# fverdoja/Fast-3D-Pointcloud-Segmentation

Measured on AMD Instinct MI355X. Metric: Mpoints/sec segmented end-to-end, 1M-pt RGB-D frames, higher is better.
Workload: dtype f32

## Files before the change

fast-3d-pointcloud-segmentation_amd/csrc/f3ds_hip.hip:

```cpp
#include <hip/hip_runtime.h>

#include <algorithm>
#include <cmath>
#include <atomic>
#include <map>
#include <chrono>
#include <cstdio>
#include <cstdlib>
#include <cstring>
#include <string>
#include <type_traits>
#include <mutex>
#include <set>
#include <vector>

#include "../../include/f3ds.h"
#include "f3ds_algo.h"
#include "f3ds_glasbey.h"
#include "f3ds_eval.h"
#include "f3ds_dev.h"
#include "f3ds_levels.h"
#include "f3ds_eval_levels.h"
#include "f3ds_rgbd.h"
#include "f3ds_track.h"
// ... 19 lines not shown
#define HIPCHECK(expr) do { hipError_t e_ = (expr); if (e_ != hipSuccess) { g_last_hip_error = std::string(#expr) + ": " + hipGetErrorString(e_); return F3DS_ERR_HIP; } } while (0)

template <class... Ts> struct ArgPack;
template <> struct ArgPack<> {};
template <class T, class... Ts> struct ArgPack<T, Ts...> { T head; ArgPack<Ts...> tail; };

template <class K, class... Done>
__device__ __forceinline__ void unpack_call(const ArgPack<>&, Done... d) { K{}(d...); }
template <class K, class T, class... Ts, class... Done>
__device__ __forceinline__ void unpack_call(const ArgPack<T, Ts...>& p, Done... d) { unpack_call<K>(p.tail, d..., p.head); }

template <class K, class = void> struct waves_per_simd { static constexpr int v = 1; };
template <class K> struct waves_per_simd<K, std::void_t<decltype(K::WAVES_PER_SIMD)>> { static constexpr int v = K::WAVES_PER_SIMD; };
template <class K, class = void> struct is_latency_kernel { static constexpr bool v = false; };
template <class K> struct is_latency_kernel<K, std::void_t<decltype(K::LATENCY_KERNEL)>> { static constexpr bool v = K::LATENCY_KERNEL; };
template <class K, class Pack>
__global__ __launch_bounds__(K::BLOCK, waves_per_simd<K>::v) void k_batched(const Pack* frames) {
#ifndef F3DS_EXP_NO_LATENCY_PRIO
    if constexpr (is_latency_kernel<K>::v) __builtin_amdgcn_s_setprio(3);
#endif
    const Pack p = frames[f3ds_frame()];
    unpack_call<K>(p);
}

template <class F> struct op_traits;
template <class C, class... Ps> struct op_traits<void (C::*)(Ps...) const> { using pack = ArgPack<std::decay_t<Ps>...>; };
template <class K> using pack_of = typename op_traits<decltype(&K::operator())>::pack;

inline void fill_pack(ArgPack<>&) {}
template <class T, class... Ts, class A, class... As>
inline void fill_pack(ArgPack<T, Ts...>& p, A a, As... as) {
    static_assert(std::is_convertible<A, T>::value && !(std::is_pointer<T>::value && std::is_integral<A>::value),
                  "rec<K>(): an argument does not convert implicitly to the kernel's parameter type (wrong element type, swapped arguments?)");
    p.head = a; fill_pack(p.tail, as...);
}

typedef hipError_t (*LaunchFn)(uint32_t gx, uint32_t nf, uint32_t lds, hipStream_t st, const void* dargs);
template <class K>
hipError_t launch_fn(uint32_t gx, uint32_t nf, uint32_t lds, hipStream_t st, const void* dargs) {
    using Pack = pack_of<K>;
    if (lds > 48u * 1024u) {
        hipError_t e = hipFuncSetAttribute(reinterpret_cast<const void*>(k_batched<K, Pack>), hipFuncAttributeMaxDynamicSharedMemorySize, (int)lds);
        if (e != hipSuccess) return e;
    }
    hipLaunchKernelGGL((k_batched<K, Pack>), dim3(gx ? gx : 1u, nf), dim3(K::BLOCK), lds, st, static_cast<const Pack*>(dargs));
    return hipGetLastError();
}
struct Cmd { LaunchFn fn; uint32_t gx, lds, bytes, off; };

const int g_inc_shift = [] { const char* e = dev_getenv("F3DS_INC_SHIFT"); return e ? atoi(e) : 6; }();

struct Switches {
    bool direct_labels = false, copy_stream = true, copy_duplex = false, split_voxel_accum = false, sweep_tiles = true, merge_spec = true, force_global_merge = false, no_stream_pool = false, sort_pairs = false, host_prof = false, trace_err = false, vox_hash = true, vox_tiles_forced = false, levels_global = false;
    int normals_threads = 0, merge_nw = 0, merge_keys = -1; uint32_t tile_holes = 0, ilist_slack = 32, r_rounds = F3DS_R_ROUNDS, grid_cap = 0, rgc_first_cap = 0; long relabel_lds_cap = -1;
    void read() {
        auto on = [](const char* n) { return dev_getenv(n) != nullptr; };
        auto num = [](const char* n, long dflt) { const char* e = dev_getenv(n); return e ? atol(e) : dflt; };
        direct_labels = num("F3DS_DIRECT_LABELS", 0) != 0; copy_stream = num("F3DS_COPY_STREAM", 1) != 0; copy_duplex = num("F3DS_COPY_STREAM", 1) == 2; split_voxel_accum = on("F3DS_SPLIT_VOXEL_ACCUM"); sweep_tiles = num("F3DS_SWEEP_TILES", 1) != 0; merge_spec = num("F3DS_MERGE_SPEC", 1) != 0;
        force_global_merge = on("F3DS_FORCE_GLOBAL_MERGE"); no_stream_pool = on("F3DS_NO_STREAM_POOL"); sort_pairs = on("F3DS_SORT_PAIRS");
        host_prof = on("F3DS_HOST_PROF"); trace_err = on("F3DS_TRACE_ERR");
        vox_tiles_forced = num("F3DS_VOX_TILES", 1) == 2;
        vox_hash = num("F3DS_VOX_TILES", 1) != 0 && !sort_pairs && !split_voxel_accum;
        normals_threads = (int)num("F3DS_NORMALS_THREADS", 0); tile_holes = (uint32_t)num("F3DS_SWEEP_TILE_HOLES", 0);
        { const long v = num("F3DS_MERGE_NW", 0); merge_nw = v == 4 ? 4 : (v ? 8 : 0); }
        { const char* e = dev_getenv("F3DS_MERGE_KEYS"); merge_keys = !e ? -1 : (!strcmp(e, "lds") ? 2 : (!strcmp(e, "global") ? 1 : 0)); }
        relabel_lds_cap = num("F3DS_RELABEL_LDS_CAP", -1);
        levels_global = num("F3DS_LEVELS_GLOBAL", 0) != 0;
        { const long v = num("F3DS_R_ROUNDS_RUN", F3DS_R_ROUNDS); r_rounds = v >= 1 && v <= F3DS_R_ROUNDS ? (uint32_t)v : (uint32_t)F3DS_R_ROUNDS; }
        { const long v = num("F3DS_ILIST_SLACK", 32); ilist_slack = v >= 1 && v <= 32 ? (uint32_t)v : 32u; }
        { const long v = num("F3DS_GRID_CAP", 0); grid_cap = v >= 1 && v <= 2048 ? (uint32_t)v : 0u; }
        { const long v = num("F3DS_RGC_FIRST_CAP", 0); rgc_first_cap = v >= 1 && v <= 0x7fffffffl ? (uint32_t)v : 0u; }
    }
};
thread_local Switches g_sw;
const int g_merge_shared_res = [] { const char* e = dev_getenv("F3DS_MERGE_SHARED_RES"); return e && atoi(e) == 2 ? 2 : 0; }();

#define F3DS_SCRATCH(X) \
    X(P16, pts)  X(unsigned char, img_depth) X(unsigned char, img_color) X(P16, spts) X(uint64_t, keys0) X(uint64_t, keys1) X(uint32_t, vals0) X(uint32_t, vals1) X(uint32_t, flags) X(uint32_t, incl) X(uint32_t, tiles) X(uint32_t, hist) X(uint32_t, seg_start) X(int, pt_voxel) X(uint32_t, labels) \
    X(uint32_t, vkey) X(uint32_t, vcount) X(float, vf) X(int, nbr) X(int, nbrT) X(uint64_t, hkeys) X(uint32_t, hvals) X(float, boxes) X(uint32_t, ckey) X(uint32_t, cell_start) X(uint64_t, chk) X(uint32_t, chv) X(uint32_t, chvals) X(int, seed_orig) X(uint32_t, keep) X(int, seed_kept) \
    X(uint32_t, owner0) X(uint32_t, ownR) X(float, dist0) X(unsigned char, R) X(float, hc) X(uint32_t, hcount) X(uint32_t, hlo) X(uint32_t, hhi) X(int, ghost_vox) X(unsigned char, ghost_active) X(unsigned char, ghost_done) X(uint32_t, ghost_head) X(uint32_t, ghost_next) \
    X(uint32_t, loff) X(float, rows) X(int, row_voxel) X(float, racc0) X(uint32_t, rcnt0) X(float, rrec0) X(unsigned char, ralive0) X(uint64_t, ehk) X(uint64_t, ekeys0) X(uint64_t, ekeys1) X(uint32_t, evals0) X(uint32_t, evals1) X(uint32_t, ea0) X(uint32_t, eb0) \
    X(uint32_t, ea) X(uint32_t, eb) X(float, ew) X(uint32_t, eku) X(int, ehist) X(unsigned char, ealive) X(uint32_t, ev_epoch) X(uint32_t, ev_key) X(int, ev_prev) X(float, racc) X(uint32_t, rcnt) X(float, rrec) X(unsigned char, ralive) X(uint32_t, rhead) X(uint32_t, rtail) X(uint32_t, lnext) X(uint32_t, parent) X(uint32_t, markA) X(uint32_t, markB) X(uint32_t, tl) X(uint32_t, merges) \
     X(float, r_vf) X(uint32_t, r_owner) X(float, r_dist) X(float, r_hc) X(uint32_t, r_hcount) X(uint32_t, r_hlo) X(uint32_t, r_hhi) X(int, r_gvox) X(unsigned char, r_gact) X(unsigned char, r_gdone) X(uint32_t, r_ghead) X(uint32_t, r_gnext) X(uint32_t, r_tl) X(uint32_t, r_tcnt) X(int, r_seed) X(uint32_t, r_L) \
    X(uint32_t, tstamp) X(uint32_t, tround) X(uint32_t, hdirty) X(uint32_t, htiles) X(uint32_t, htcnt) X(uint32_t, vwl) X(uint32_t, vwl2) X(uint32_t, vtmask) \
     X(uint32_t, glut) X(uint32_t, truth_pts) X(uint32_t, tsum) X(uint32_t, tcol) X(uint32_t, tlab) X(uint32_t, ctab) X(uint32_t, csize) X(uint32_t, eroot) X(uint32_t, eincl) \
     X(uint32_t, hcnt) X(uint32_t, pslot) X(uint32_t, vlist) \
     X(uint32_t, u_src) X(uint32_t, u_voff) X(float, u_xyz) X(uint32_t, u_rgba) X(float, u_cent) X(float, u_nrm) \
    X(float, deltas) X(uint64_t, skeys0) X(uint64_t, skeys1) X(uint32_t, svals0) X(uint32_t, svals1) X(uint32_t, cdf_hist) X(float, cdf) X(uint32_t, root) X(uint32_t, rincl) X(uint32_t, rrank) X(uint2, pool) X(uint32_t, rstart) X(uint32_t, rnleaf) X(uint32_t, rcap) X(uint32_t, tile_n1) X(uint32_t, tile_ord) X(uint32_t, tile_slots) X(uint32_t, ilist) X(uint32_t, istart) X(uint32_t, ilen) X(uint32_t, icap) \
     X(uint32_t, lv_into) X(uint32_t, lv_at) X(uint32_t, lv_pfx) X(float, lv_thr) X(uint32_t, lv_tab) X(uint32_t, lv_nreg) X(uint32_t, lv_out) \
     \
    X(uint64_t, evl_k0) X(uint64_t, evl_k1) X(uint32_t, evl_v0) X(uint32_t, evl_v1) X(uint32_t, evl_flag) X(uint64_t, evl_bkey) X(uint32_t, evl_bcnt) X(uint64_t, evl_ukey) X(uint32_t, evl_ucnt) X(uint32_t, evl_glist) \
    X(uint32_t, evl_ssize) X(unsigned char, evl_used) X(float, evl_hterm) X(float, evl_mterm) X(float, evl_tterm) X(uint32_t, evl_tsize) X(uint32_t, evl_order) X(uint32_t, evl_slot) X(uint32_t, evl_counts) X(uint32_t, evl_out) \
     \
    X(uint32_t, trk_lab) X(uint32_t, trk_end) X(uint32_t, trk_out) X(uint32_t, trk_id) X(uint32_t, trk_tid) \
     \
    X(unsigned char, rgt_depth) X(unsigned char, rgt_color) X(uint32_t, rgt_lab) X(RgAcc, rgt_acc) X(unsigned char, rgt_out) \
     \
    X(unsigned char, rgc_depth) X(uint32_t, rgc_lab) X(uint64_t, rgc_k0) X(uint64_t, rgc_k1) X(uint32_t, rgc_v0) X(uint32_t, rgc_v1) X(uint32_t, rgc_rec) X(uint32_t, rgc_flag) X(uint64_t, rgc_ukey) X(uint32_t, rgc_ustart) X(uint32_t, rgc_uend) X(uint32_t, rgc_cnt) X(unsigned char, rgc_out) \
     \
    X(unsigned char, rgs_depth) X(uint32_t, rgs_lab) X(ShAcc, rgs_acc) X(unsigned char, rgs_out) \
     \
    X(unsigned char, rgk_depth) X(uint32_t, rgk_lab) X(uint32_t, rgk_parent) X(uint32_t, rgk_cnt) X(uint32_t, rgk_flag) X(unsigned char, rgk_out)
template <class T> struct Scratch { T* p = nullptr; size_t cap = 0; int slot = -1; };
#define F3DS_SCRATCH_SLOT(T, name) S_##name,
#define F3DS_SCRATCH_MEMBER(T, name) Scratch<T> name{nullptr, 0, S_##name};
#define F3DS_SCRATCH_VISIT(T, name) if (const int rc_ = f(name)) return rc_;
enum ScratchSlot { F3DS_SCRATCH(F3DS_SCRATCH_SLOT) N_SCRATCH };

}

struct f3ds_ctx {
    int device = 0;
    hipStream_t own_stream = nullptr;
    hipStream_t stream = nullptr;
    hipEvent_t ev[11] = {};
    DevCounters* d_dc = nullptr;
    DevCounters* h_dc = nullptr;
    GridInfo* d_grid = nullptr;
    GridInfo* h_grid = nullptr;
    SeedGrid* d_sgrid = nullptr;
    std::vector<Cmd> cmds;
    std::vector<unsigned char> blob;
    std::vector<uintptr_t> pend;
// ... 482 lines not shown
    } else {
        rec<d_helper_own>(c, grid_for(S0, 256), 0u, sb.seeds, S0, owner0);
        rec<d_helper_init>(c, grid_for(S0 + 1, 256), 0u, sb.seeds, S0, owner0, ghost_vox, ghost_active, ghost_done, hlo, hhi, hcount, hc, tl, tcnt);
    }
    const int* nbrT = c->nbrT.p; const float* vf = sb.vf;
    SweepFrame a;
    a.sv = SweepView{(int)V, nbrT, vf, owner0, dist0, hc, ghost_head, ghost_next, &c->d_dc->n_ghosts, prm.seed_res, prm.w_normal, prm.w_color, prm.w_spatial, c->nbr.p};
    a.R = R; a.ownR = ownR; a.owner_out = owner0; a.dist_out = dist0;
    a.ghost_done = ghost_done; a.ghost_active = ghost_active; a.ghost_vox = ghost_vox; a.ghost_head = ghost_head; a.ghost_next = ghost_next;
    a.hlo = hlo; a.hhi = hhi; a.hcount = hcount; a.hc = hc; a.dc = c->d_dc; a.S0 = S0;
    a.tR0 = tiles4; a.tR1 = tiles4 + T; a.tC0 = tiles4 + 2 * (size_t)T; a.tC1 = tiles4 + 3 * (size_t)T; a.tRr = trr; a.hD = hD; a.T = T; a.tl = tl; a.tcnt = tcnt; a.wl = wl; a.wl2 = wl2; a.tmask = tmask;
    a.thr = a_sweep_thr(V, g_inc_shift);
    if (!g_sw.sweep_tiles) a.tile_n1 = nullptr;
    else a.tile_n1 = c->tile_n1.p;
    a.tile_ord = c->tile_ord.p; a.tile_slots = c->tile_slots.p;
    for (uint32_t t = 0; t < c->res.sweeps; ++t) {
        if (a_sweep_needs_clear(t)) rec_fill(c, R, 0u, V);
        rec<d_sweep_begin>(c, 1u, 0u, a, t);
        const bool can_skip = t >= 2u;
        const bool rounds = g_inc_shift >= 0 && can_skip;
        const uint32_t nrounds = rounds ? g_sw.r_rounds : 0u;
        rec<d_sweep_R_first>(c, grid_for(V, 256), 0u, a, a_sweep_tag(t), t, nrounds);
        for (uint32_t r = 1; r < nrounds; ++r) rec<d_sweep_R_round>(c, grid_for(V, 256), 0u, a, t, r, nrounds);
        for (uint32_t pass = 0; pass < F3DS_R_PASSES; ++pass) rec<d_sweep_R>(c, pass == 0 ? grid_for(V, 256) : 64u, 0u, a, a_sweep_tag(t), t, pass);
        rec<d_sweep_R_tail>(c, 1u, 0u, a, a_sweep_tag(t), t);
        rec<d_sweep_claim>(c, grid_for(V, 256), 0u, a, t);
        rec<d_centroid>(c, grid_for((size_t)S0 * 64u, 256), 0u, a, t);
    }
    return F3DS_OK;
}
int seg_sweeps(f3ds_ctx* c) {
    SweepBufs sb{&c->owner0, &c->dist0, &c->hc, &c->hcount, &c->hlo, &c->hhi, &c->ghost_vox, &c->ghost_active, &c->ghost_done, &c->ghost_head, &c->ghost_next, &c->htiles, &c->htcnt, c->vf.p, c->seed_kept.p, false};
    return seg_sweeps_on(c, sb);
}
int seg_supervoxels(f3ds_ctx* c) {
    const uint32_t V = c->V, S0 = c->S0;
    uint32_t *loff, *rcnt0, *ev0, *ev1; float *rows, *racc0, *rrec0; int* row_voxel; unsigned char* ralive0; uint64_t *ehk, *ek0, *ek1;
    ENSURE(c->loff, S0 + 2, loff);
    int rc = scan_u32(c, c->hcount.p, loff + 1, S0 + 1);
    if (rc) return rc;
    rec_fill(c, loff, 0u, 4);
    ENSURE(c->rows, ((size_t)V + S0 + 1) * 12, rows); ENSURE(c->row_voxel, (size_t)V + S0 + 1, row_voxel);
    ENSURE(c->racc0, (size_t)(S0 + 1) * 12, racc0); ENSURE(c->rcnt0, S0 + 1, rcnt0); ENSURE(c->rrec0, (size_t)(S0 + 1) * 16, rrec0);
    ENSURE(c->ralive0, S0 + 1, ralive0);
    rec_fill(c, ralive0, 0u, S0 + 1);
    rec_fill(c, rcnt0, 0u, (size_t)(S0 + 1) * 4);
    rec<d_sv_fill>(c, S0 ? (S0 + 3u) / 4u : 1u, 0u,
                   c->vf.p, c->owner0.p, S0, c->hlo.p, c->hhi.p, c->ghost_vox.p, c->ghost_active.p, c->hcount.p, loff, c->hc.p, rows, row_voxel, racc0, rcnt0, rrec0, ralive0, c->d_dc, c->htiles.p, c->htcnt.p, V);
    const uint32_t ecap = (uint32_t)std::min<uint64_t>((uint64_t)S0 * c->edge_mult + 1024u, 0x7fffffffu);
    const uint32_t ehcap = pow2_ge((size_t)ecap * 2);
    ENSURE(c->ehk, ehcap, ehk);
    ENSURE(c->ekeys0, ecap, ek0); ENSURE(c->ekeys1, ecap, ek1); ENSURE(c->evals0, ecap, ev0); ENSURE(c->evals1, ecap, ev1);
    rec_fill(c, ehk, 0xFFFFFFFFu, (size_t)ehcap * 8);
    rec<d_edges>(c, grid_for(V, 256), 0u, V, S0, c->nbrT.p, c->owner0.p, ehk, ehcap - 1, ek0, ecap, c->d_dc);
    rec<d_edges_ghost>(c, grid_for(S0, 256), 0u, V, S0, c->ghost_vox.p, c->ghost_active.p, c->nbrT.p, c->owner0.p, ehk, ehcap - 1, ek0, ecap, c->d_dc);
    return F3DS_OK;
}
int seg_edge_sort(f3ds_ctx* c, int sort_bits) {
    const uint32_t E = c->E, S0 = c->S0;
    uint32_t *ea0, *eb0; ENSURE(c->ea0, E, ea0); ENSURE(c->eb0, E, eb0);
    uint32_t* evs;
    { uint32_t* h; ENSURE(c->hist, (size_t)RS_BINS * (((size_t)E * 2 + RS_TILE - 1) / RS_TILE + 1), h); }
    rec<d_iota>(c, grid_for(E, 256), 0u, c->evals0.p, E);
    int rc = radix_sort(c, c->ekeys0.p, c->evals0.p, c->ekeys1.p, c->evals1.p, E, sort_bits, &c->eks, &evs);
    if (rc) return rc;
    rec<d_edge_init>(c, grid_for(E, 256), 0u, c->eks, E, S0, ea0, eb0);
    return F3DS_OK;
}
bool merge_il_layout(uint32_t E, uint32_t S0, int nw, int res, MergeLds* xl) {
    memset(xl, 0, sizeof *xl);
    if ((uint64_t)E * (res == 2 ? 10u : 2u) > (1u << 22)) return false;
    const MergeIlLayout L = merge_il_offsets(E, nw, res);
    xl->Ecap = L.Ecap; xl->NGcap = L.NGcap; xl->lds_bytes = L.total; xl->keys_in_lds = res;
    xl->spec = g_sw.merge_spec ? 1 : 0;
    return L.total <= MC_LDS_LIMIT && S0 <= 65534u;
}
enum MergeKind { MK_GLOBAL = 0, MK_IL = 1 };
inline int mk_waves(int kind) { return (kind - MK_IL) >= 2 ? 4 : 8; }
inline int mk_res(int kind) { return (kind - MK_IL) % 2 ? 0 : 2; }
int choose_merge_kind(const std::vector<f3ds_ctx*>& fr, bool force_global) {
    if (force_global || g_sw.force_global_merge) return MK_GLOBAL;
    const bool e_keys = g_sw.merge_keys >= 0;
    const bool shared = fr.size() >= 16 && g_batch_calls[fr[0]->device & 15].load(std::memory_order_relaxed) >= 2;
    const int nw = g_sw.merge_nw ? (g_sw.merge_nw == 8 ? 8 : 4) : (shared ? 4 : 8);
    const int first = e_keys ? (g_sw.merge_keys == 2 ? 2 : 0) : (shared ? g_merge_shared_res : 2);
    for (int res = first; res >= (e_keys ? first : 0); res -= 2) {
        bool ok = true;
        for (f3ds_ctx* c : fr) { MergeLds t; if (!merge_il_layout(c->E, c->S0, nw, res, &t)) { ok = false; break; } }
        if (ok) return MK_IL + (nw == 8 ? 0 : 2) + (res == 2 ? 0 : 1);
    }
    return MK_GLOBAL;
}
int seg_cluster_front(f3ds_ctx* c, const f3ds_params* prm, int kind) {
    const bool use_lds = kind != MK_GLOBAL;
    const uint32_t S0 = c->S0, E = c->E;
    float lambda = 0.5f; int bins = 500;
    if (prm->merging == F3DS_MANUAL_LAMBDA && prm->lambda != 0) { if (prm->lambda < 0 || prm->lambda > 1) return F3DS_ERR_RANGE; lambda = prm->lambda; }
    if (prm->merging == F3DS_EQUALIZATION && prm->bins != 0) { if (prm->bins < 0) return F3DS_ERR_RANGE; bins = (short)prm->bins; }
    if (prm->merging < 0 || prm->merging > 2 || prm->color_metric < 0 || prm->color_metric > 1 || prm->geom_metric < 0 || prm->geom_metric > 1) return F3DS_ERR_ARG;
    MergeDev m;
    memset(&m, 0, sizeof m);
    m.E = E; m.S0 = S0; m.threshold = prm->threshold; m.dc = c->d_dc;
    { const uint64_t cap = (uint64_t)E * c->ev_mult + 4096u; m.ev_cap = cap > 0x7fffffffull ? 0x7fffffffu : (uint32_t)cap; }
    ENSURE(c->ea, E, m.ea); ENSURE(c->eb, E, m.eb); ENSURE(c->ew, ((size_t)E + 2047) & ~(size_t)2047, m.ew);  ENSURE(c->eku, ((size_t)E + 2047) & ~(size_t)2047, m.eku);
    ENSURE(c->ehist, E, m.ehist); ENSURE(c->ealive, E, m.ealive);
    ENSURE(c->ev_epoch, m.ev_cap, m.ev_epoch); ENSURE(c->ev_key, m.ev_cap, m.ev_key); ENSURE(c->ev_prev, m.ev_cap, m.ev_prev);
    ENSURE(c->racc, (size_t)(S0 + 1) * 12, m.racc); ENSURE(c->rrec, (size_t)(S0 + 1) * 16, m.rrec);
    ENSURE(c->rcnt, S0 + 1, m.rcnt); ENSURE(c->ralive, S0 + 1, m.ralive);
// ... 1793 lines not shown
```

fast-3d-pointcloud-segmentation_amd/csrc/f3ds_kernels.inc:

```


namespace {

struct P16 { float x, y, z; uint32_t rgba; };

struct DevCounters {
    unsigned long long n_finite;
    uint32_t bbox[6];
    uint32_t bbox_any;
    uint32_t n_valid;
    uint32_t n_voxels;
    uint32_t n_cells;
    uint32_t n_seeds;
    uint32_t n_edges;
    uint32_t n_alive;
    uint32_t n_merges;
    uint32_t n_regions;
    uint32_t n_events;
    int error;
    int r_overflow;
    float lambda;
    uint32_t seg_count;
    uint32_t n_ghosts;
    int depth;
// ... 1784 lines not shown
            }
            __syncthreads();
        }
        if (threadIdx.x == 0) seed[h - 1u] = sv[0];
    }
};
struct d_reseed_own {
    static constexpr int BLOCK = 256;
    __device__ void operator()(const int* seed, uint32_t S0, uint32_t* owner) const {
        for (uint32_t i = BIX * blockDim.x + threadIdx.x; i < S0; i += gridDim.x * blockDim.x) if (seed[i] >= 0) atomicMax(&owner[seed[i]], i + 1u);
    }
};
struct d_reseed_init {
    static constexpr int BLOCK = 256;
    __device__ void operator()(const int* seed, uint32_t S0, const uint32_t* owner, int* ghost_vox, unsigned char* ghost_active, unsigned char* ghost_done, uint32_t* hlo,
                               uint32_t* hhi, uint32_t* hcount, uint32_t* tl, uint32_t* tcnt) const {
        for (uint32_t i = BIX * blockDim.x + threadIdx.x; i <= S0; i += gridDim.x * blockDim.x) {
            ghost_done[i] = 0;
            const int v = i == 0u ? -1 : seed[i - 1];
            if (v < 0) { ghost_vox[i] = -1; ghost_active[i] = 0; hlo[i] = 0; hhi[i] = 0; hcount[i] = 0; tcnt[i] = 0; continue; }
            const bool ghost = owner[v] != i;
            ghost_vox[i] = ghost ? v : -1;
            ghost_active[i] = ghost ? 1 : 0;
            hlo[i] = (uint32_t)v; hhi[i] = (uint32_t)v; hcount[i] = 1;
            tl[(size_t)i * HT_CAP] = (uint32_t)v >> 6; tcnt[i] = ghost ? 0u : 1u;
        }
    }
};
struct SweepFrame {
    SweepView sv;
    unsigned char* R; uint32_t* ownR;
    uint32_t* owner_out; float* dist_out;
    unsigned char *ghost_done, *ghost_active; int* ghost_vox; uint32_t *ghost_head, *ghost_next;
    uint32_t *hlo, *hhi, *hcount; float* hc; DevCounters* dc; uint32_t S0;
    uint32_t *tR0, *tR1, *tC0, *tC1;
    uint32_t* tRr;
    uint32_t* hD;
    uint32_t *tl, *tcnt;
    uint32_t *wl, *wl2;
    uint32_t* tmask;
    uint32_t T, thr;
    const uint32_t *tile_n1, *tile_ord, *tile_slots;
    __device__ uint32_t* tR_this(uint32_t t) const { return (t & 1u) ? tR1 : tR0; }
    __device__ uint32_t* tC_this(uint32_t t) const { return (t & 1u) ? tC1 : tC0; }
    __device__ uint32_t* tR_next(uint32_t t) const { return (t & 1u) ? tR0 : tR1; }
    __device__ uint32_t* tC_next(uint32_t t) const { return (t & 1u) ? tC0 : tC1; }
};
template <bool ROWS = false>
__device__ inline void mark_tiles(const SweepView& s, int v, uint32_t* a, uint32_t* b, uint32_t stamp) {
#pragma unroll
    for (int k0 = 0; k0 < 27; k0 += 9) {
        int nu[9];
#pragma unroll
        for (int k = 0; k < 9; ++k) nu[k] = ROWS ? a_nbr_w(s, v, k0 + k) : a_nbr(s, v, k0 + k);
#pragma unroll
        for (int k = 0; k < 9; ++k) {
            const int u = nu[k] >= 0 ? nu[k] : v;
            a[u >> 6] = stamp; b[u >> 6] = stamp;
        }
    }
}
struct d_sweep_begin {
    static constexpr bool LATENCY_KERNEL = true;
    static constexpr int BLOCK = 256;
    __device__ void operator()(SweepFrame f, uint32_t t) const {
        __shared__ uint32_t s_n;
        if (threadIdx.x == 0) s_n = 0;
        for (uint32_t h = 1 + threadIdx.x; h <= f.S0; h += blockDim.x) if (f.ghost_vox[h] >= 0) f.ghost_head[f.ghost_vox[h]] = 0u;
        __syncthreads();
        uint32_t mine = 0;
        for (uint32_t h = 1 + threadIdx.x; h <= f.S0; h += blockDim.x)
            if (f.ghost_active[h]) { f.ghost_next[h] = atomicExch(&f.ghost_head[f.ghost_vox[h]], h); mine++; }
        if (mine) atomicAdd(&s_n, mine);
        __syncthreads();
        if (threadIdx.x == 0) {
            f.dc->n_ghosts = s_n;
            if (t == 0u) f.dc->sweep_stats[0] = f.dc->sweep_stats[1] = f.dc->sweep_stats[2] = f.dc->sweep_stats[3] = 0u;
            if (!a_sweep_begin(sweep_ctl(f.dc), t, s_n, f.thr)) { f.dc->sweep_stats[F3DS_SWEEP_IDLE]++; return; }
            for (int p = 0; p <= F3DS_R_PASSES; ++p) f.dc->rq[p] = 0u;
        }
    }
};
struct SweepTile {
    uint32_t (*lds)[NT_RING1 + 1];
    uint32_t (*lds2)[NT_RING1 + 1];
    int half, li;
    static constexpr int SR = (NT_RING1 + NT_TILE - 1) / NT_TILE;
    __device__ bool stage(const SweepFrame& f, uint32_t tl, const uint32_t* src, const uint32_t* src2) {
        uint32_t n1 = SW_TILE_NONE;
        if (f.tile_n1 && tl * (uint32_t)NT_TILE < (uint32_t)f.sv.V) n1 = f.tile_n1[tl];
        const bool tiled = n1 != SW_TILE_NONE;
        uint32_t a[SR], b[SR];
        if (tiled) {
            const uint32_t* ord = f.tile_ord + (size_t)tl * NT_RING1;
            uint32_t u[SR];
#pragma unroll
            for (int k = 0; k < SR; ++k) { const uint32_t i = (uint32_t)(li + k * NT_TILE); u[k] = ord[i < n1 ? i : 0u]; }
#pragma unroll
            for (int k = 0; k < SR; ++k) a[k] = src[u[k]];
            if (src2) {
#pragma unroll
                for (int k = 0; k < SR; ++k) b[k] = src2[u[k]];
            }
        }
        __syncthreads();
        if (tiled) {
#pragma unroll
// ... 143 lines not shown
            if (n == 0u) break;
            const uint32_t* src = (q & 1u) ? f.wl2 : f.wl;
            uint32_t* dst = (q & 1u) ? f.wl : f.wl2;
            for (uint32_t i = threadIdx.x; i < n; i += blockDim.x) {
                const uint32_t e = src[i];
                const int v = (int)(e & 0x7fffffffu);
                int overflow = 0;
                const uint32_t o = s.owner[v];
                const bool r = masks ? a_eval_R_mask(s, v, f.R, tag, f.tmask, &overflow) : a_eval_R(s, v, f.R, tag, &overflow, false);
                if (!overflow) f.ownR[v] = o | (r ? F3DS_OWNR_RTRUE : 0u);
                else dst[atomicAdd(&s_next, 1u)] = e;
            }
            __threadfence();
            __syncthreads();
            if (threadIdx.x == 0) { if (s_next == n) f.dc->r_overflow = 1; s_n = s_next == n ? 0u : s_next; s_next = 0; }
            __syncthreads();
        }
    }
};
struct d_sweep_R_round {
    static constexpr int BLOCK = 256;
    static constexpr int WAVES_PER_SIMD = 6;
    __device__ void operator()(SweepFrame f, uint32_t t, uint32_t r, uint32_t nrounds) const {
        const SweepCtl ctl = sweep_ctl(f.dc);
        if (a_sweep_is_full(ctl, t) || a_sweep_is_idle(ctl, t)) return;
        __shared__ uint32_t nown[2][NT_RING1 + 1];
        const SweepView s = f.sv;
        const uint32_t stamp = t + 1u;
        const uint32_t* cur = r == 0u ? f.tR_this(t) : f.tRr + (size_t)(r - 1u) * f.T;
        const bool last = r + 1u == nrounds;
        uint32_t* tc = f.tC_this(t);
        uint32_t* nxt = last ? tc : f.tRr + (size_t)r * f.T;
        SweepTile st{nown, nown, (int)(threadIdx.x >> 7), (int)(threadIdx.x & 127u)};
        __shared__ uint32_t s_marked[2];
        const uint32_t bix = BIX, step = gridDim.x;
        for (uint32_t tp0 = bix; tp0 * 256u < (uint32_t)s.V; tp0 += 64u * step)
          for (uint64_t marked = marked_pairs(cur, stamp, tp0, step, (uint32_t)s.V, s_marked); marked; marked &= marked - 1ull) {
            const uint32_t tp = tp0 + (uint32_t)__builtin_ctzll(marked) * step;
            const uint32_t tl = tp * 2u + (uint32_t)st.half;
            const int v = (int)(tl * (uint32_t)NT_TILE) + st.li;
            const bool active = v < s.V && cur[v >> 6] == stamp;
            const bool tiled = st.stage_held(f, tl);
            if (!active) continue;
            const uint32_t o = s.owner[v];
            bool keeps;
            if (tiled) {
                uint32_t og[27];
                st.gather(f, tl, og, nullptr);
                keeps = o != 0u && !a_has_thief_words(s, v, o, og);
            } else keeps = a_eval_R_step(s, f.ownR, v);
            const uint32_t nw = o | (keeps ? F3DS_OWNR_RTRUE : 0u);
            if (nw != f.ownR[v]) {
                f.ownR[v] = nw;
                mark_tiles(s, v, nxt, tc, stamp);
                if (last) a_sweep_turn_full(ctl, t);
            }
        }
    }
};
#ifndef F3DS_RFIRST_WPS
#define F3DS_RFIRST_WPS 6
#endif
struct d_sweep_R_first {
    static constexpr int BLOCK = 256;
    static constexpr int WAVES_PER_SIMD = F3DS_RFIRST_WPS;
    __device__ void operator()(SweepFrame f, unsigned char tag, uint32_t t, uint32_t rounds) const {
        d_sweep_R_pre{}(f, tag, t);
        if (rounds) d_sweep_R_round{}(f, t, 0u, rounds);
    }
};
struct d_sweep_claim {
    static constexpr int BLOCK = 256;
    __device__ void operator()(SweepFrame f, uint32_t t) const {
        __shared__ uint32_t nr[2][NT_RING1 + 1], ngh[2][NT_RING1 + 1];
        const SweepCtl ctl = sweep_ctl(f.dc);
        if (a_sweep_is_idle(ctl, t)) return;
        const SweepView s = f.sv;
        const bool full = a_sweep_is_full(ctl, t);
        const bool marks = a_sweep_marks(ctl, t);
        const bool ghosts = *s.n_ghosts != 0u;
        const uint32_t* cur = f.tC_this(t);
        uint32_t changed = 0;
        SweepTile st{nr, ngh, (int)(threadIdx.x >> 7), (int)(threadIdx.x & 127u)};
        __shared__ uint32_t s_marked[2];
        const uint32_t bix = BIX, step = gridDim.x;
        for (uint32_t tp0 = bix; tp0 * 256u < (uint32_t)s.V; tp0 += 64u * step) {
          uint64_t marked = ~0ull;
          if (!full) marked = marked_pairs(cur, t + 1u, tp0, step, (uint32_t)s.V, s_marked);
          for (; marked; marked &= marked - 1ull) {
            const uint32_t tp = tp0 + (uint32_t)__builtin_ctzll(marked) * step;
            if (tp * 256u >= (uint32_t)s.V) break;
            const uint32_t tl = tp * 2u + (uint32_t)st.half;
            const int v = (int)(tl * (uint32_t)NT_TILE) + st.li;
            const bool active = v < s.V && (full || cur[v >> 6] == t + 1u);
            const bool tiled = st.stage(f, tl, f.ownR, ghosts ? s.ghost_head : nullptr);
            if (!active) continue;
            uint32_t o; float d;
            bool plain = false;
            if (tiled) {
                uint32_t cand[27];
                bool near = false;
                st.gather(f, tl, cand, ghosts ? &near : nullptr);
                if (!near) {
                    a_claim_words(s, v, cand, &o, &d);
                    plain = true;
                }
            }
            if (!plain) a_claim(s, f.ownR, v, &o, &d, f.ghost_done);
            const uint32_t o0 = s.owner[v];
            bool gained = false;
            if (o != o0 || __float_as_uint(d) != __float_as_uint(s.dist[v])) {
                f.owner_out[v] = o; f.dist_out[v] = d;
                if (o != o0) {
                    gained = o != 0u;
                    if (o0 != 0u) f.hD[o0] = t + 1u;
                }
                if (marks) mark_tiles(s, v, f.tR_next(t), f.tC_next(t), t + 2u);
                changed++;
            }
            for (uint64_t todo = __ballot(gained); todo;) {
                const int first = __builtin_ctzll(todo);
                const uint32_t og = (uint32_t)__builtin_amdgcn_readlane((int)o, first);
                const uint64_t peers = __ballot(gained && o == og);
                if (lane_id() == first) {
                    const uint32_t vmax = (uint32_t)v + (uint32_t)(63 - __builtin_clzll(peers)) - (uint32_t)first;
                    atomicMin(&f.hlo[og], (uint32_t)v); atomicMax(&f.hhi[og], vmax); f.hD[og] = t + 1u;
                    const uint32_t pos = atomicAdd(&f.tcnt[og], 1u);
                    if (pos < HT_CAP) f.tl[(size_t)og * HT_CAP + pos] = (uint32_t)v >> 6;
                }
                todo &= ~peers;
            }
          }
        }
    #pragma unroll
        for (int d = 32; d >= 1; d >>= 1) changed += __shfl_xor(changed, d, 64);
        if (lane_id() == 0 && changed) atomicAdd(ctl.n_changed, changed);
    }
};
__device__ inline int helper_tile_list(const uint32_t* tl, uint32_t cnt, int gv, uint32_t* srt) {
    const uint32_t n = cnt + (gv >= 0 ? 1u : 0u);
    if (cnt > HT_CAP) return -1;
    const uint32_t lane = (uint32_t)lane_id();
    if (n <= 64u) {
        uint32_t tid = 0xFFFFFFFFu;
        if (lane < cnt) tid = tl[lane];
        else if (lane == cnt && gv >= 0) tid = (uint32_t)gv >> 6;
        bool dup = lane >= n;
        for (uint32_t j = 0; j + 1u < n; ++j) { const uint32_t tj = __builtin_amdgcn_readlane(tid, j); if (j < lane && tj == tid) dup = true; }
        const uint64_t keep = __ballot(!dup);
        uint32_t rank = 0;
        for (uint64_t m = keep; m; m &= m - 1ull) { const uint32_t tj = __builtin_amdgcn_readlane(tid, (uint32_t)__builtin_ctzll(m)); rank += tj < tid; }
        if (!dup) srt[rank] = tid;
        wave_lds_sync();
        return __popcll(keep);
    }
    uint32_t nd = 0;
    for (uint32_t base = 0; base < n; base += 64u) {
        const uint32_t idx = base + lane;
        uint32_t tid = 0xFFFFFFFFu;
        if (idx < cnt) tid = tl[idx];
        else if (idx == cnt && gv >= 0) tid = (uint32_t)gv >> 6;
        bool dup = idx >= n;
        for (uint32_t j = 0; j < 64u; ++j) { const uint32_t tj = __builtin_amdgcn_readlane(tid, j); if (j < lane && tj == tid) dup = true; }
        for (uint32_t j = 0; j < nd; ++j) if (srt[j] == tid) dup = true;
        const uint64_t keep = __ballot(!dup);
        const uint32_t k = (uint32_t)__popcll(keep);
        if (nd + k > 64u) return -1;
        wave_lds_sync();
        if (!dup) srt[nd + (uint32_t)__popcll(keep & lanemask_lt())] = tid;
        nd += k;
// ... 472 lines not shown
        float acc = 0.0f;
        for (uint32_t done = 0; done < len; done += 64u) {
            const uint32_t nbuf = len - done < 64u ? len - done : 64u;
            wave_lds_sync();
            if ((uint32_t)lane < nbuf) {
                const uint32_t v = off + done + (uint32_t)lane;
                const float x = vxyz[(size_t)v * 3], y = vxyz[(size_t)v * 3 + 1], z = vxyz[(size_t)v * 3 + 2];
                const uint32_t c = vrgba[v];
                const float row[12] = {x * x, x * y, x * z, y * y, y * z, z * z, x, y, z, (float)((c >> 16) & 255u), (float)((c >> 8) & 255u), (float)(c & 255u)};
        #pragma unroll
                for (int k = 0; k < 12; ++k) { pay[lane][k] = row[k]; rows[(size_t)v * 12 + k] = row[k]; }
                row_voxel[v] = (int)v; owner[v] = h;
            }
            wave_lds_sync();
            if (lane < 12) for (uint32_t j = 0; j < nbuf; ++j) {
                const float r = pay[j][lane];
                if (lane < 9) acc += r;
                else { const float count = (float)(done + j + 1u); const float inv = 1 / count; acc = acc + inv * (r - acc); }
            }
        }
        if (lane < 12) racc0[(size_t)h * 12 + lane] = acc;
        const float mr = __shfl(acc, 9, 64), mg = __shfl(acc, 10, 64), mb = __shfl(acc, 11, 64);
        float lab[3];
        lab_three_lanes(lane == 0 ? mr : (lane == 1 ? mg : mb), lane, lab);
        if (lane == 0) {
            rcnt0[h] = len; ralive0[h] = 1;
            atomicAdd(&dc->n_alive, 1u);
            float rec[16];
            rec[0] = cxyz[(size_t)i * 3]; rec[1] = cxyz[(size_t)i * 3 + 1]; rec[2] = cxyz[(size_t)i * 3 + 2];
            rec[3] = cnrm[(size_t)i * 3]; rec[4] = cnrm[(size_t)i * 3 + 1]; rec[5] = cnrm[(size_t)i * 3 + 2];
            rec[6] = mr; rec[7] = mg; rec[8] = mb;
            rec[9] = lab[0]; rec[10] = lab[1]; rec[11] = lab[2];
            rec[12] = rec[13] = rec[14] = rec[15] = 0.0f;
            for (int k = 0; k < 16; ++k) rrec0[(size_t)h * 16 + k] = rec[k];
            float* c12 = hc + (size_t)h * 12;
            c12[0] = rec[0]; c12[1] = rec[1]; c12[2] = rec[2]; c12[3] = mr; c12[4] = mg; c12[5] = mb; c12[6] = rec[3]; c12[7] = rec[4]; c12[8] = rec[5]; c12[9] = c12[10] = c12[11] = 0.0f;
        }
    }
};
__device__ inline void edge_insert(uint64_t key, uint64_t* hkeys, uint32_t hmask, uint64_t* ekeys, uint32_t ecap, DevCounters* dc) {
    uint32_t hh = (uint32_t)hash64(key) & hmask;
    for (uint32_t probes = 0; probes <= hmask; ++probes) {
        unsigned long long old = atomicCAS((unsigned long long*)&hkeys[hh], (unsigned long long)HASH_EMPTY, (unsigned long long)key);
        if (old == key) return;
        if (old == HASH_EMPTY) {
            uint32_t pos = atomicAdd(&dc->n_edges, 1u);
            if (pos < ecap) ekeys[pos] = key; else { dc->error = F3DS_ERR_UNSUPPORTED; dc->ev_overflow = 3; }
            return;
        }
        hh = (hh + 1u) & hmask;
    }
    dc->error = F3DS_ERR_UNSUPPORTED;
}
__device__ inline void leaf_edges(uint32_t h, uint32_t v, uint32_t V, uint32_t S0, const int* nbrT, const uint32_t* owner, uint64_t* hkeys, uint32_t hmask,
                                  uint64_t* ekeys, uint32_t ecap, DevCounters* dc) {
    int nu[27]; uint32_t og[27];
#pragma unroll
    for (int s = 0; s < 27; ++s) nu[s] = nbrT[(size_t)s * V + v];
#pragma unroll
    for (int s = 0; s < 27; ++s) {
        const uint32_t o = owner[nu[s] >= 0 ? (uint32_t)nu[s] : v];
        og[s] = (nu[s] >= 0 && o && o != h && h < o) ? o : 0u;
    }
    uint32_t last = 0;
#pragma unroll
    for (int s = 0; s < 27; ++s) {
        const uint32_t o = og[s];
        if (o && o != last) { last = o; edge_insert((uint64_t)h * (S0 + 1ull) + o, hkeys, hmask, ekeys, ecap, dc); }
    }
}
struct d_edges {
    static constexpr int BLOCK = 256;
    __device__ void operator()(uint32_t V, uint32_t S0, const int* nbrT, const uint32_t* owner, uint64_t* hkeys, uint32_t hmask,
                                              uint64_t* ekeys, uint32_t ecap, DevCounters* dc) const {
        for (uint32_t v = BIX * blockDim.x + threadIdx.x; v < V; v += gridDim.x * blockDim.x) {
            const uint32_t h = owner[v];
            if (h) leaf_edges(h, v, V, S0, nbrT, owner, hkeys, hmask, ekeys, ecap, dc);
        }
    }
};
struct d_edges_ghost {
    static constexpr int BLOCK = 256;
    __device__ void operator()(uint32_t V, uint32_t S0, const int* ghost_vox, const unsigned char* ghost_active, const int* nbrT,
                                                    const uint32_t* owner, uint64_t* hkeys, uint32_t hmask, uint64_t* ekeys, uint32_t ecap, DevCounters* dc) const {
        for (uint32_t h = 1 + BIX * blockDim.x + threadIdx.x; h <= S0; h += gridDim.x * blockDim.x)
            if (ghost_active[h]) leaf_edges(h, (uint32_t)ghost_vox[h], V, S0, nbrT, owner, hkeys, hmask, ekeys, ecap, dc);
    }
};
struct d_iota {
    static constexpr int BLOCK = 256;
    __device__ void operator()(uint32_t* v, uint32_t n) const {
        for (uint32_t i = BIX * blockDim.x + threadIdx.x; i < n; i += gridDim.x * blockDim.x) v[i] = i;
    }
};
struct d_fill_f32 {
    static constexpr int BLOCK = 256;
    __device__ void operator()(float* v, uint32_t n, float x) const {
        for (uint32_t i = BIX * blockDim.x + threadIdx.x; i < n; i += gridDim.x * blockDim.x) v[i] = x;
    }
};
struct d_edge_init {
    static constexpr int BLOCK = 256;
    __device__ void operator()(const uint64_t* ekeys, uint32_t E, uint32_t S0, uint32_t* ea0, uint32_t* eb0) const {
        for (uint32_t e = BIX * blockDim.x + threadIdx.x; e < E; e += gridDim.x * blockDim.x) {
            ea0[e] = (uint32_t)(ekeys[e] / (S0 + 1ull)); eb0[e] = (uint32_t)(ekeys[e] % (S0 + 1ull));
        }
    }
};
struct d_edge_deltas {
    static constexpr int BLOCK = 256;
    __device__ void operator()(uint32_t E, const uint32_t* ea, const uint32_t* eb, const float* rrec, int color_metric, int geom_metric,
                                                    float* deltas, uint64_t* skeys, uint32_t* svals) const {
        for (uint32_t e = BIX * blockDim.x + threadIdx.x; e < E; e += gridDim.x * blockDim.x) {
            float dc_, dg_;
            n_delta_c_g(rrec + (size_t)ea[e] * 16, rrec + (size_t)eb[e] * 16, color_metric, geom_metric, &dc_, &dg_);
            deltas[e * 2] = dc_; deltas[e * 2 + 1] = dg_;
            if (skeys) {
                skeys[e] = (uint64_t)n_weight_key(dc_); svals[e] = e * 2u;
                skeys[E + e] = (1ull << 32) | (uint64_t)n_weight_key(dg_); svals[E + e] = e * 2u + 1u;
            }
        }
    }
};
struct d_lambda {
    static constexpr bool LATENCY_KERNEL = true;
    static constexpr int BLOCK = 64;
    __device__ void operator()(uint32_t E, const float* deltas, const uint32_t* svals, DevCounters* dc) const {
        const int lane = lane_id();
        float count = 0, mean_d = 0;
        for (uint32_t base = 0; base < E; base += 64u) {
            const uint32_t i = base + lane;
            const float vc = i < E ? deltas[svals[i]] : 0.0f;
            const float vg = i < E ? deltas[svals[(size_t)E + i]] : 0.0f;
            const int nb = E - base < 64u ? (int)(E - base) : 64;
            const float inv = 1 / (count + (float)(lane + 1));
    #pragma unroll
            for (int j = 0; j < 64; ++j) {
                if (j < nb) {
                    const float dcj = __builtin_bit_cast(float, __builtin_amdgcn_readlane(__builtin_bit_cast(int, vc), j));
// ... 1271 lines not shown
```

Measured before the change: 3735.

## Deduplicate supervoxel edges in a per-block LDS set before global hash insert

The edge-extraction kernel now stages neighbour owners through the sweep-tile shared-memory path where tiles exist, and enumerates distinct higher-labelled neighbours via a next-label scan. Candidate edge keys go first into a per-block LDS hash set, which is flushed to the global edge hash table in rounds. The aim is to cut global atomicCAS contention and duplicate probes, since many voxels in a block share the same supervoxel pairs. The cost is extra block-wide syncs and flush loops. The ghost kernel and the ROWS path switch from the transposed neighbour array to row-major nbr.

```diff
diff --git a/fast-3d-pointcloud-segmentation_amd/csrc/f3ds_hip.hip b/fast-3d-pointcloud-segmentation_amd/csrc/f3ds_hip.hip
--- a/fast-3d-pointcloud-segmentation_amd/csrc/f3ds_hip.hip
+++ b/fast-3d-pointcloud-segmentation_amd/csrc/f3ds_hip.hip
@@ -95,7 +95,7 @@
 
 struct Switches {
     bool direct_labels = false, copy_stream = true, copy_duplex = false, split_voxel_accum = false, sweep_tiles = true, merge_spec = true, force_global_merge = false, no_stream_pool = false, sort_pairs = false, host_prof = false, trace_err = false, vox_hash = true, vox_tiles_forced = false, levels_global = false;
-    int normals_threads = 0, merge_nw = 0, merge_keys = -1; uint32_t tile_holes = 0, ilist_slack = 32, r_rounds = F3DS_R_ROUNDS, grid_cap = 0, rgc_first_cap = 0; long relabel_lds_cap = -1;
+    int normals_threads = 0, merge_nw = 0, merge_keys = -1; uint32_t tile_holes = 0, ilist_slack = 32, r_rounds = F3DS_R_ROUNDS, grid_cap = 0, rgc_first_cap = 0, edge_set = ES_CAP; long relabel_lds_cap = -1;
     void read() {
         auto on = [](const char* n) { return dev_getenv(n) != nullptr; };
         auto num = [](const char* n, long dflt) { const char* e = dev_getenv(n); return e ? atol(e) : dflt; };
@@ -112,6 +112,7 @@
         { const long v = num("F3DS_R_ROUNDS_RUN", F3DS_R_ROUNDS); r_rounds = v >= 1 && v <= F3DS_R_ROUNDS ? (uint32_t)v : (uint32_t)F3DS_R_ROUNDS; }
         { const long v = num("F3DS_ILIST_SLACK", 32); ilist_slack = v >= 1 && v <= 32 ? (uint32_t)v : 32u; }
         { const long v = num("F3DS_GRID_CAP", 0); grid_cap = v >= 1 && v <= 2048 ? (uint32_t)v : 0u; }
+        { const long v = num("F3DS_EDGE_SET", ES_CAP); edge_set = v >= (long)ES_CAP_MIN && v <= (long)ES_CAP && !(v & (v - 1)) ? (uint32_t)v : ES_CAP; }
         { const long v = num("F3DS_RGC_FIRST_CAP", 0); rgc_first_cap = v >= 1 && v <= 0x7fffffffl ? (uint32_t)v : 0u; }
     }
 };
@@ -700,8 +701,8 @@
     ENSURE(c->ehk, ehcap, ehk);
     ENSURE(c->ekeys0, ecap, ek0); ENSURE(c->ekeys1, ecap, ek1); ENSURE(c->evals0, ecap, ev0); ENSURE(c->evals1, ecap, ev1);
     rec_fill(c, ehk, 0xFFFFFFFFu, (size_t)ehcap * 8);
-    rec<d_edges>(c, grid_for(V, 256), 0u, V, S0, c->nbrT.p, c->owner0.p, ehk, ehcap - 1, ek0, ecap, c->d_dc);
-    rec<d_edges_ghost>(c, grid_for(S0, 256), 0u, V, S0, c->ghost_vox.p, c->ghost_active.p, c->nbrT.p, c->owner0.p, ehk, ehcap - 1, ek0, ecap, c->d_dc);
+    rec<d_edges>(c, grid_for(V, 256), 0u, V, S0, c->nbr.p, c->owner0.p, g_sw.sweep_tiles ? c->tile_n1.p : nullptr, c->tile_ord.p, c->tile_slots.p, g_sw.edge_set, ehk, ehcap - 1, ek0, ecap, c->d_dc);
+    rec<d_edges_ghost>(c, grid_for(S0, 256), 0u, S0, c->ghost_vox.p, c->ghost_active.p, c->nbr.p, c->owner0.p, ehk, ehcap - 1, ek0, ecap, c->d_dc);
     return F3DS_OK;
 }
 int seg_edge_sort(f3ds_ctx* c, int sort_bits) {
diff --git a/fast-3d-pointcloud-segmentation_amd/csrc/f3ds_kernels.inc b/fast-3d-pointcloud-segmentation_amd/csrc/f3ds_kernels.inc
--- a/fast-3d-pointcloud-segmentation_amd/csrc/f3ds_kernels.inc
+++ b/fast-3d-pointcloud-segmentation_amd/csrc/f3ds_kernels.inc
@@ -1860,7 +1860,7 @@
     for (int k0 = 0; k0 < 27; k0 += 9) {
         int nu[9];
 #pragma unroll
-        for (int k = 0; k < 9; ++k) nu[k] = ROWS ? a_nbr_w(s, v, k0 + k) : a_nbr(s, v, k0 + k);
+        for (int k = 0; k < 9; ++k) nu[k] = ROWS ? s.nbr_rows[(size_t)v * 27u + (size_t)(k0 + k)] : a_nbr(s, v, k0 + k);
 #pragma unroll
         for (int k = 0; k < 9; ++k) {
             const int u = nu[k] >= 0 ? nu[k] : v;
@@ -2110,7 +2110,7 @@
             const uint32_t nw = o | (keeps ? F3DS_OWNR_RTRUE : 0u);
             if (nw != f.ownR[v]) {
                 f.ownR[v] = nw;
-                mark_tiles(s, v, nxt, tc, stamp);
+                mark_tiles<true>(s, v, nxt, tc, stamp);
                 if (last) a_sweep_turn_full(ctl, t);
             }
         }
@@ -2173,7 +2173,7 @@
                     gained = o != 0u;
                     if (o0 != 0u) f.hD[o0] = t + 1u;
                 }
-                if (marks) mark_tiles(s, v, f.tR_next(t), f.tC_next(t), t + 2u);
+                if (marks) mark_tiles<true>(s, v, f.tR_next(t), f.tC_next(t), t + 2u);
                 changed++;
             }
             for (uint64_t todo = __ballot(gained); todo;) {
@@ -2752,39 +2752,86 @@
     }
     dc->error = F3DS_ERR_UNSUPPORTED;
 }
-__device__ inline void leaf_edges(uint32_t h, uint32_t v, uint32_t V, uint32_t S0, const int* nbrT, const uint32_t* owner, uint64_t* hkeys, uint32_t hmask,
-                                  uint64_t* ekeys, uint32_t ecap, DevCounters* dc) {
-    int nu[27]; uint32_t og[27];
-#pragma unroll
-    for (int s = 0; s < 27; ++s) nu[s] = nbrT[(size_t)s * V + v];
-#pragma unroll
-    for (int s = 0; s < 27; ++s) {
-        const uint32_t o = owner[nu[s] >= 0 ? (uint32_t)nu[s] : v];
-        og[s] = (nu[s] >= 0 && o && o != h && h < o) ? o : 0u;
-    }
-    uint32_t last = 0;
-#pragma unroll
-    for (int s = 0; s < 27; ++s) {
-        const uint32_t o = og[s];
-        if (o && o != last) { last = o; edge_insert((uint64_t)h * (S0 + 1ull) + o, hkeys, hmask, ekeys, ecap, dc); }
+constexpr uint32_t EP_DONE = 0xFFFFFFFFu;
+template <class Put>
+__device__ inline uint32_t leaf_pairs(uint32_t h, uint32_t S0, const uint32_t x[27], uint32_t last, Put put) {
+    for (;;) {
+        const uint32_t y = a_next_label(x, last + 1u);
+        if (y >= F3DS_NO_NEXT) return EP_DONE;
+        const uint32_t o = y + last + 1u;
+        if (!put((uint64_t)h * (S0 + 1ull) + o)) return last;
+        last = o;
     }
 }
+__device__ inline void row_owners(const int* nbr, const uint32_t* owner, uint32_t v, uint32_t x[27]) {
+    int nu[27];
+#pragma unroll
+    for (int k = 0; k < 27; ++k) nu[k] = nbr[(size_t)v * 27u + (uint32_t)k];
+#pragma unroll
+    for (int k = 0; k < 27; ++k) {
+        const uint32_t o = owner[nu[k] >= 0 ? (uint32_t)nu[k] : v];
+        x[k] = nu[k] >= 0 ? o : 0u;
+    }
+}
+#ifndef F3DS_EDGE_SET
+#define F3DS_EDGE_SET 512
+#endif
+constexpr uint32_t ES_CAP = F3DS_EDGE_SET;
+constexpr uint32_t ES_CAP_MIN = 4;
+static_assert(ES_CAP >= ES_CAP_MIN && (ES_CAP & (ES_CAP - 1u)) == 0u, "the edge set's capacity is a power of two");
 struct d_edges {
     static constexpr int BLOCK = 256;
-    __device__ void operator()(uint32_t V, uint32_t S0, const int* nbrT, const uint32_t* owner, uint64_t* hkeys, uint32_t hmask,
-                                              uint64_t* ekeys, uint32_t ecap, DevCounters* dc) const {
-        for (uint32_t v = BIX * blockDim.x + threadIdx.x; v < V; v += gridDim.x * blockDim.x) {
-            const uint32_t h = owner[v];
-            if (h) leaf_edges(h, v, V, S0, nbrT, owner, hkeys, hmask, ekeys, ecap, dc);
+    __device__ void operator()(uint32_t V, uint32_t S0, const int* nbr, const uint32_t* owner, const uint32_t* tile_n1, const uint32_t* tile_ord, const uint32_t* tile_slots,
+                               uint32_t cap, uint64_t* hkeys, uint32_t hmask, uint64_t* ekeys, uint32_t ecap, DevCounters* dc) const {
+        __shared__ uint32_t nown[2][NT_RING1 + 1];
+        __shared__ unsigned long long set[ES_CAP];
+        SweepFrame f{};
+        f.sv.V = (int)V; f.tile_n1 = tile_n1; f.tile_ord = tile_ord; f.tile_slots = tile_slots;
+        SweepTile st{nown, nown, (int)(threadIdx.x >> 7), (int)(threadIdx.x & 127u)};
+        for (uint32_t e = threadIdx.x; e < cap; e += 256u) set[e] = HASH_EMPTY;
+        auto put = [&](uint64_t key) {
+            uint32_t e = (uint32_t)hash64(key) & (cap - 1u);
+            for (uint32_t probes = 0; probes < cap; ++probes) {
+                const unsigned long long old = atomicCAS(&set[e], (unsigned long long)HASH_EMPTY, (unsigned long long)key);
+                if (old == HASH_EMPTY || old == key) return true;
+                e = (e + 1u) & (cap - 1u);
+            }
+            return false;
+        };
+        for (uint32_t tp = BIX; tp * 256u < V; tp += gridDim.x) {
+            const uint32_t tl = tp * 2u + (uint32_t)st.half;
+            const uint32_t v = tl * (uint32_t)NT_TILE + (uint32_t)st.li;
+            const bool tiled = st.stage(f, tl, owner, nullptr);
+            const uint32_t h = v < V ? owner[v] : 0u;
+            uint32_t x[27];
+            uint32_t last = EP_DONE;
+            if (h) {
+                if (tiled) st.gather(f, tl, x, nullptr); else row_owners(nbr, owner, v, x);
+                last = h;
+            }
+            for (;;) {
+                if (last != EP_DONE) last = leaf_pairs(h, S0, x, last, put);
+                const int more = __syncthreads_or(last != EP_DONE);
+                for (uint32_t e = threadIdx.x; e < cap; e += 256u) {
+                    const unsigned long long key = set[e];
+                    if (key != HASH_EMPTY) { edge_insert(key, hkeys, hmask, ekeys, ecap, dc); set[e] = HASH_EMPTY; }
+                }
+                if (!more) break;
+                __syncthreads();
+            }
         }
     }
 };
 struct d_edges_ghost {
     static constexpr int BLOCK = 256;
-    __device__ void operator()(uint32_t V, uint32_t S0, const int* ghost_vox, const unsigned char* ghost_active, const int* nbrT,
+    __device__ void operator()(uint32_t S0, const int* ghost_vox, const unsigned char* ghost_active, const int* nbr,
                                                     const uint32_t* owner, uint64_t* hkeys, uint32_t hmask, uint64_t* ekeys, uint32_t ecap, DevCounters* dc) const {
         for (uint32_t h = 1 + BIX * blockDim.x + threadIdx.x; h <= S0; h += gridDim.x * blockDim.x)
-            if (ghost_active[h]) leaf_edges(h, (uint32_t)ghost_vox[h], V, S0, nbrT, owner, hkeys, hmask, ekeys, ecap, dc);
+            if (ghost_active[h]) {
+                uint32_t x[27];
+                row_owners(nbr, owner, (uint32_t)ghost_vox[h], x);
+                leaf_pairs(h, S0, x, h, [&](uint64_t key) { edge_insert(key, hkeys, hmask, ekeys, ecap, dc); return true; });
+            }
     }
 };
 struct d_iota {
```

Measured after the change: 3766, median of 6. Within noise of the previous version (+0.8%).
